# Pablete1234/parquet-floor

Measured on AMD Instinct MI355X. Metric: decoded GB/s + rows/s (node), lineitem-shape Snappy+dict, 1/2/4/8 GPUs, higher is better.
Workload: dtype u8; 1 GPU; lineitem SF1 x1 (6001215 rows x 1, 16 cols, 6 row groups of 1Mi rows), Snappy + dictionary, device-resident; row_groups_per_rank=6, compressed_page_bytes_rank0=217870360

## Files before the change

### parquet-floor_amd/csrc/pf_internal.h

```cpp
#pragma once
#include <stdint.h>

#include "pf_page_tables.h"

namespace pf {

struct Int2 {
    int x, y;
};

struct PfOpts {
    int exec = 5;
    bool ba_fused = true;
    bool page_null = false;
    int null_stagger = 0;
    bool nest_timeout = false;
    uint32_t null_dcap = 0;
    unsigned debug_skip = 0;
    int force_serial = 0;
    int force_redo = 0;
    bool zc = true;
    bool dl_kernel = true;
    bool h2d_kernel = false;
    int h2d_grid = 256;
    bool dl_stream = true;
    bool dl_prio = false;
    bool debug_plan = false;
    int64_t nest_seg = 0;
    bool nest_seg_set = false;
    bool dbp_par = true;
    bool bloom_first = true;
    bool flat_dstr = true;
    int fix_shift = 1;
};

constexpr uint32_t BA_TILE = 8192;
constexpr uint64_t BA_SHORT = 48;
constexpr uint32_t STICKY_DICT = 64u << 10;
constexpr uint32_t SNAP_RB = 128;
constexpr uint32_t SNAP_WIN = 64 * SNAP_RB;
constexpr uint32_t SNAP_WWORDS = SNAP_WIN / 32;
constexpr uint32_t SNAP_BLOCK = 65536;

struct SnapWin {
    uint32_t entry;
    uint32_t exit;
    uint32_t out;
    uint32_t flags;
};

struct SnapEnt {
    uint32_t pos;
    uint32_t out;
};

enum : int32_t {
    PG_V2 = 1,
    PG_COMPRESSED = 2,
    PG_DICT = 4,
};

struct SnappyJob {
    const uint8_t* src;
    uint8_t* dst;
    uint32_t src_len;
// ... 257 lines not shown
```

### parquet-floor_amd/csrc/pf_launch.h

```cpp
#pragma once
#include <hip/hip_runtime.h>

#include "pf_internal.h"
#include "pfloor.h"

namespace pf {

void launch_snappy_serial(const SnappyJob* d_jobs, int n_jobs, const int* d_fallback, DevChunkResult* d_res, hipStream_t s);
void launch_snappy_parse(const SnappyJob* d_jobs, int n_jobs, const int2* d_wins, int n_wins, SnapWin* d_win, SnapEnt* d_ent,
                         uint32_t* d_lane_out, uint32_t* d_splits, int* d_fb, int max_nwin, hipStream_t s);
void launch_snappy_exec(const SnappyJob* d_jobs, int n_jobs, const int2* d_pieces, int n_pieces, uint32_t* d_splits, int* d_fb,
                        DevChunkResult* d_res, int exec, hipStream_t s);
void launch_snappy(const SnappyJob* d_jobs, int n_jobs, const int2* d_wins, int n_wins, SnapWin* d_win, SnapEnt* d_ent,
                   uint32_t* d_lane_out, const int2* d_pieces, int n_pieces, uint32_t* d_splits, int* d_fb,
                   DevChunkResult* d_res, int max_nwin, int exec, hipStream_t s);
#ifdef PF_DIAG
void launch_snappy_exec2(const SnappyJob* d_jobs, int n_jobs, const int2* d_pieces, int n_pieces, const uint32_t* d_splits,
                         int* d_fb, hipStream_t s);
#endif

void launch_zstd(ZstdJob* d_jobs, const int* d_order, int n_jobs, uint8_t* d_lit, uint32_t lit_stride, DevChunkResult* d_res,
                 hipStream_t s);

void launch_lz4(Lz4Job* d_jobs, const int* d_order, int n_jobs, DevChunkResult* d_res, hipStream_t s);

void launch_snappy_head(SnappyJob* d_jobs, int n_jobs, DevPage* d_pages, const DevChunk* d_chunks, int* d_fb,
                        const DevChunkResult* d_res, hipStream_t st);
void launch_snappy_litcopy(const SnappyJob* d_jobs, const int* d_list, int n, const int* d_fb, hipStream_t st);

void launch_ba(BaJob* d_jobs, int n_jobs, const int2* d_tiles, int n_tiles, DevChunkResult* d_res, hipStream_t st,
               bool short_values);

void launch_runs(const DevChunk* d_chunks, DevPage* d_pages, const int* d_list, int n, DevChunkResult* d_res, hipStream_t st);
void launch_lvl(const DevChunk* d_chunks, DevPage* d_pages, const int* d_list, int n, DevChunkResult* d_res, hipStream_t st,
                bool page_null, NullCaps nc);
void launch_count_flat(const DevChunk* d_chunks, DevPage* d_pages, const int* d_list, int n, int n_flat, const int2* d_dblk,
                       int n_dblk, DevChunkResult* d_res, BaJob* d_bajobs, hipStream_t st);
void launch_flat(const DevChunk* d_chunks, DevPage* d_pages, const int* d_list, int nfix, int n, int n4, int n8, int* d_fbq,
                 const int2* d_dblk, int n_dblk, DevChunkResult* d_res, hipStream_t st, NullCaps nc, int stagger);

void launch_nest_lvl(const DevChunk* d_chunks, DevPage* d_pages, const int* d_list, int n, int max_nwin, DevChunkResult* d_res,
                     hipStream_t st, bool force_timeout);
void launch_count(const DevChunk* d_chunks, DevPage* d_pages, const int* d_list, int n, DevChunkResult* d_res, BaJob* d_bajobs,
                  hipStream_t st, int idle_grid);
void launch_nest_count(const DevChunk* d_chunks, DevPage* d_pages, const int* d_list, int n, const int2* d_segs, int n_segs,
                       DevChunkResult* d_res, hipStream_t st);
void launch_scan(DevChunk* d_chunks, DevPage* d_pages, const int* d_list, int n, DevChunkResult* d_res, uint8_t* arena,
                 uint64_t cap, unsigned long long* used, hipStream_t st);
// ... 24 lines not shown
```

### parquet-floor_amd/csrc/pf_runtime.hip

```cpp
#include <hip/hip_runtime.h>

#include <algorithm>
#include <chrono>
#include <cstdio>
#include <cstdlib>
#include <cstring>
#include <memory>
#include <mutex>
#include <string>
#include <vector>

#include "pf_ctx.h"
#include "pf_host.h"
#include "pf_launch.h"
#include "pf_plan.h"
#include "pf_snappy_par.h"
#include "pfloor.h"

using namespace pf;

static_assert(sizeof(Int2) == sizeof(int2) && alignof(Int2) <= alignof(int2), "the planner's pairs are the kernels' int2");

namespace {

// ... 68 lines not shown
    hipStream_t st = ctx->stream;
    const BatchPlan& p = ctx->plan;
    uint8_t* meta = static_cast<uint8_t*>(ctx->d_meta.p);
    DevChunk* d_chunks = reinterpret_cast<DevChunk*>(meta + p.off_chunks);
    DevPage* d_pages = reinterpret_cast<DevPage*>(meta + p.off_pages);
    SnappyJob* d_jobs = reinterpret_cast<SnappyJob*>(meta + p.off_jobs);
    DevChunkResult* d_res = reinterpret_cast<DevChunkResult*>(meta + p.off_res);
    auto list = [&](ListId l) { return reinterpret_cast<int*>(meta + p.off_lists) + p.list_base[l]; };
    auto pairs = [&](ListId l) { return reinterpret_cast<const int2*>(list(l)); };
    auto len = [&](ListId l) { return int(p.lists[l].size()); };
    const int n_jobs = int(p.jobs.size()), n_nest = len(L_NEST), n_nseg = len(L_NSEG) / 2;
    unsigned long long* used = reinterpret_cast<unsigned long long*>(meta + p.meta_bytes - 256);
    const int2* d_pieces = reinterpret_cast<const int2*>(meta + p.off_pieces);
    uint32_t* d_splits = reinterpret_cast<uint32_t*>(meta + p.off_splits);
    int* d_fallback = reinterpret_cast<int*>(meta + p.off_fallback);
    const int2* d_wins = reinterpret_cast<const int2*>(meta + p.off_wins);

#ifdef PF_DIAG
    const unsigned skip = ctx->opts.debug_skip;
#else
    constexpr unsigned skip = 0;
#endif
    if (!ctx->meta_by_kernel) {
        if (p.bits_bytes) HIPCHK(ctx, hipMemsetAsync(ctx->d_bits.p, 0, p.bits_bytes, st));
        if (p.npub_bytes) HIPCHK(ctx, hipMemsetAsync(static_cast<uint8_t*>(ctx->d_scratch.p) + p.off_npub, 0, p.npub_bytes, st));
    }
    EVREC(ctx, ctx->ev[1], st);
    if (!(skip & 1u)) launch_snappy_head(d_jobs, n_jobs, d_pages, d_chunks, d_fallback, d_res, st);
    if (!(skip & 1u)) launch_snappy_litcopy(d_jobs, list(L_DJOBS), len(L_DJOBS), d_fallback, st);
    if (!(skip & 1u)) launch_snappy_parse(d_jobs, n_jobs, d_wins, int(p.snap.wins.size()), p.snap.d_win, p.snap.d_ent,
                        p.snap.d_lane_out, d_splits, d_fallback, p.snap.max_snap_win, st);
    EVREC(ctx, ctx->ev[2], st);
    if (!(skip & 2u))
        launch_snappy_exec(d_jobs, n_jobs, d_pieces, int(p.snap.pieces.size()), d_splits, d_fallback, d_res, ctx->opts.exec, st);
    launch_zstd(reinterpret_cast<ZstdJob*>(meta + p.off_zjobs), list(L_ZSTD), int(p.zjobs.size()),
                static_cast<uint8_t*>(ctx->d_scratch.p) + p.off_zlit, p.zlit_stride, d_res, st);
    launch_lz4(reinterpret_cast<Lz4Job*>(meta + p.off_ljobs), list(L_LZ4), int(p.ljobs.size()), d_res, st);
    EVREC(ctx, ctx->ev[3], st);
    BaJob* d_bajobs = reinterpret_cast<BaJob*>(meta + p.off_bajobs);
    const int2* d_batiles = reinterpret_cast<const int2*>(meta + p.off_batiles);
    const int n_ba = int(p.bajobs.size()), n_bt = int(p.ba_tiles.size());
    if (!(skip & 4u)) launch_ba(d_bajobs, p.n_ba_dict, d_batiles, p.n_ba_dict_tiles, d_res, st, p.ba_short_dict && ctx->opts.ba_fused);
    EVREC(ctx, ctx->ev[4], st);
    launch_delta(d_chunks, d_pages, list(L_DELTA), len(L_DELTA), p.max_dbp_nwin, d_res, st);
    EVREC(ctx, ctx->ev[5], st);
    if (!(skip & 8u)) launch_runs(d_chunks, d_pages, list(L_RUNS), len(L_RUNS), d_res, st);
    NullCaps ncaps = p.null_caps;
    if (ctx->opts.null_dcap) ncaps.dcap = ctx->opts.null_dcap;
    if (!(skip & 8u)) launch_lvl(d_chunks, d_pages, list(L_LVL), len(L_LVL), d_res, st, ctx->opts.page_null, ncaps);
    launch_dlen(d_chunks, d_pages, list(L_DLEN), len(L_DLEN), d_res, st);
    EVREC(ctx, ctx->ev[6], st);
    launch_nest_lvl(d_chunks, d_pages, list(L_NEST), n_nest, p.max_nwin, d_res, st, ctx->opts.nest_timeout);
    if (!(skip & 16u)) {
        launch_count_flat(d_chunks, d_pages, list(L_COUNT), len(L_COUNT), p.n_count_flat, pairs(L_CDICT), len(L_CDICT) / 2,
                          d_res, d_bajobs, st);
        launch_count(d_chunks, d_pages, list(L_COUNT), len(L_COUNT), d_res, d_bajobs, st, COUNT_IDLE_GRID);
    }
    launch_nest_count(d_chunks, d_pages, list(L_NEST), n_nest, pairs(L_NSEG), n_nseg, d_res, st);
    if (!(skip & 4u))
        launch_ba(d_bajobs + p.n_ba_dict, n_ba - p.n_ba_dict, d_batiles + p.n_ba_dict_tiles, n_bt - p.n_ba_dict_tiles,
                  d_res, st, p.ba_short_data && ctx->opts.ba_fused);
    EVREC(ctx, ctx->ev[7], st);
    launch_scan(d_chunks, d_pages, list(L_SCAN), len(L_SCAN), d_res, static_cast<uint8_t*>(ctx->d_chars.p),
                ctx->d_chars.cap, used, st);
    EVREC(ctx, ctx->ev[8], st);
    if (!(skip & 32u))
        launch_flat(d_chunks, d_pages, list(L_FLAT), p.n_flat_fixed, p.n_flat_all, p.n_null4, p.n_null8,
// ... 126 lines not shown

namespace {
#ifdef PF_DIAG
void opts_from_env(pf::PfOpts& o) {
    auto on = [](const char* name, bool dflt) { const char* e = std::getenv(name); return e ? e[0] == '1' : dflt; };
    auto num = [](const char* name, int dflt) { const char* e = std::getenv(name); return e ? std::atoi(e) : dflt; };
    o.exec = num("PF_EXEC", o.exec);
    o.ba_fused = on("PF_BA_FUSED", o.ba_fused);
    o.page_null = on("PF_PAGE_NULL", o.page_null);
    o.nest_timeout = on("PF_DEBUG_NEST_TIMEOUT", o.nest_timeout);
    o.null_dcap = uint32_t(std::max(0, num("PF_NULL_DCAP", 0))) & ~15u;
    o.null_stagger = num("PF_DEBUG_NULL_STAGGER", o.null_stagger);
    if (const char* e = std::getenv("PF_DEBUG_SKIP")) {
        const char* names[] = {"parse", "exec", "ba", "levels", "count", "flat", "decode"};
        for (int i = 0; i < 7; i++)
            if (std::strstr(e, names[i])) o.debug_skip |= 1u << i;
    }
    o.force_serial = num("PF_DEBUG_FORCE_SERIAL", o.force_serial);
    o.force_redo = num("PF_DEBUG_FORCE_REDO", o.force_redo);
    o.zc = on("PF_ZC", o.zc);
    o.dl_kernel = on("PF_DL_KERNEL", o.dl_kernel);
    o.dl_stream = on("PF_DL_STREAM", o.dl_stream);
    o.h2d_kernel = on("PF_H2D_KERNEL", o.h2d_kernel);
    o.h2d_grid = std::max(1, num("PF_H2D_GRID", o.h2d_grid));
    o.dl_prio = on("PF_DL_PRIO", o.dl_prio);
    o.debug_plan = on("PF_DEBUG_PLAN", o.debug_plan);
    if (const char* e = std::getenv("PF_NEST_SEG")) {
        o.nest_seg = std::atoll(e);
        o.nest_seg_set = true;
    }
    o.dbp_par = on("PF_DBP_PAR", o.dbp_par);
    o.bloom_first = on("PF_BLOOM_FIRST", o.bloom_first);
    o.flat_dstr = on("PF_FLAT_DSTR", o.flat_dstr);
    const int fb = num("PF_FIX_BLK", 8192);
    o.fix_shift = fb >= 16384 ? 2 : (fb >= 8192 ? 1 : 0);
}
#endif

int ctx_init(pf_ctx* ctx, pf_ctx* peer) {
#ifdef PF_DIAG
    opts_from_env(ctx->opts);
#endif
    HIPCHK(nullptr, hipSetDevice(ctx->device));
    if (peer) {
        ctx->streams = peer->streams;
    } else {
        ctx->streams = std::make_shared<Streams>();
        ctx->streams->device = ctx->device;
        HIPCHK(nullptr, hipStreamCreateWithFlags(&ctx->streams->stream, hipStreamNonBlocking));
    }
    ctx->stream = ctx->streams->stream;
    ctx->zc = ctx->opts.zc;
    HIPCHK(nullptr, hipEventCreateWithFlags(&ctx->ev_done, hipEventDisableTiming));
    HIPCHK(nullptr, hipEventCreateWithFlags(&ctx->ev_copy, hipEventDisableTiming));
    HIPCHK(nullptr, hipEventCreateWithFlags(&ctx->ev_dl, hipEventDisableTiming));
    for (auto& e : ctx->ev) HIPCHK(nullptr, hipEventCreate(&e));
    for (auto& e : ctx->ev_bloom) HIPCHK(nullptr, hipEventCreate(&e));
    for (auto& e : ctx->ev_win) HIPCHK(nullptr, hipEventCreate(&e));
    for (auto& e : ctx->ev_sel) HIPCHK(nullptr, hipEventCreate(&e));
    return PF_OK;
}

int ctx_create(int device, pf_ctx* peer, pf_ctx** out) {
    pf_ctx* ctx = new pf_ctx();
    ctx->device = device;
    const int rc = ctx_init(ctx, peer);
// ... 495 lines not shown
    SnappyJob job{};
    job.src = static_cast<const uint8_t*>(ctx->d_in.p);
    job.dst = static_cast<uint8_t*>(ctx->d_scratch.p);
    job.src_len = uint32_t(n);
    job.dst_len = uint32_t(ulen);
    std::vector<SnappyJob> jobs(1, job);
    SnappyPlan sp;
    plan_snappy(jobs, sp);
    HIPCHK(ctx, ctx->d_tokmap.ensure(sp.tokmap_bytes));
    bind_snappy(jobs, sp, reinterpret_cast<uintptr_t>(ctx->d_tokmap.p));
    ctx->d_last_win = sp.d_win;
    ctx->d_last_lane_out = sp.d_lane_out;
    size_t m = 0;
    auto take = [](size_t& cursor, size_t sz) { size_t o = align_up(cursor, 256); cursor = o + sz; return o; };
    size_t o_job = take(m, sizeof(SnappyJob)), o_pc = take(m, sizeof(int2) * sp.pieces.size());
    size_t o_sp = take(m, 4 * sp.pieces.size()), o_fb = take(m, 4), o_wn = take(m, sizeof(int2) * sp.wins.size());
    size_t o_res = take(m, sizeof(DevChunkResult));
    m = align_up(m, 256);
    HIPCHK(ctx, ctx->d_meta.ensure(m));
    HIPCHK(ctx, ctx->h_meta.ensure(m));
    uint8_t* h = static_cast<uint8_t*>(ctx->h_meta.p);
    std::memset(h, 0, m);
    std::memcpy(h + o_job, jobs.data(), sizeof(SnappyJob));
    std::memcpy(h + o_pc, sp.pieces.data(), sizeof(int2) * sp.pieces.size());
    std::memset(h + o_sp, 0xff, 4 * sp.pieces.size());
    std::memcpy(h + o_wn, sp.wins.data(), sizeof(int2) * sp.wins.size());
    uint8_t* d = static_cast<uint8_t*>(ctx->d_meta.p);
    HIPCHK(ctx, hipMemcpyAsync(d, h, m, hipMemcpyHostToDevice, st));
    ctx->d_last_splits = reinterpret_cast<const uint32_t*>(d + o_sp);
    launch_snappy(reinterpret_cast<const SnappyJob*>(d + o_job), 1, reinterpret_cast<const int2*>(d + o_wn),
                  int(sp.wins.size()), sp.d_win, sp.d_ent, sp.d_lane_out, reinterpret_cast<const int2*>(d + o_pc),
                  int(sp.pieces.size()), reinterpret_cast<uint32_t*>(d + o_sp), reinterpret_cast<int*>(d + o_fb),
                  reinterpret_cast<DevChunkResult*>(d + o_res), int(jobs[0].n_win),
                  ctx->opts.exec, st);
    HIPCHK(ctx, hipGetLastError());
    HIPCHK(ctx, ctx->h_res.ensure(512));
    HIPCHK(ctx, hipMemcpyAsync(ctx->h_res.p, d + o_res, sizeof(DevChunkResult), hipMemcpyDeviceToHost, st));
    HIPCHK(ctx, hipMemcpyAsync(static_cast<uint8_t*>(ctx->h_res.p) + 256, d + o_fb, 4, hipMemcpyDeviceToHost, st));
    if (ulen) HIPCHK(ctx, hipMemcpyAsync(dst, ctx->d_scratch.p, ulen, hipMemcpyDeviceToHost, st));
    HIPCHK(ctx, hipStreamSynchronize(st));
    const DevChunkResult* r = static_cast<const DevChunkResult*>(ctx->h_res.p);
    if (r->status != 0) return fail(ctx, r->status, "snappy: corrupt input");
    return PF_OK;
}

int pf_zstd_decompress(pf_ctx* ctx, const uint8_t* src, size_t n, uint8_t* dst, size_t cap, size_t* out_len) {
    if (!ctx || (!src && n) || (!dst && cap) || !out_len) return fail(ctx, PF_ERR_INVALID_ARG, "null arg");
    if (ctx->pending) return fail(ctx, PF_ERR_STATE, "previous decode not waited for");
    if (n > (1ull << 30) || cap > (1ull << 30)) return fail(ctx, PF_ERR_INVALID_ARG, "zstd: buffer too large");
    *out_len = 0;
    if (const int rc = begin_oneshot(ctx, true)) return rc;
    hipStream_t st = ctx->stream;
    const uint32_t stride = zstd_lit_stride(uint32_t(cap));
    const size_t o_lit = align_up(cap + 16, 256);
    HIPCHK(ctx, ctx->d_in.ensure(std::max<size_t>(n, 1)));
    HIPCHK(ctx, ctx->d_scratch.ensure(o_lit + stride));
    if (n) HIPCHK(ctx, hipMemcpyAsync(ctx->d_in.p, src, n, hipMemcpyHostToDevice, st));
    ZstdJob job{};
    job.src = static_cast<const uint8_t*>(ctx->d_in.p);
    job.dst = static_cast<uint8_t*>(ctx->d_scratch.p);
    job.src_len = uint32_t(n);
    job.dst_len = uint32_t(cap);
    const size_t o_res = 256, m = 512;
    HIPCHK(ctx, ctx->d_meta.ensure(m));
    HIPCHK(ctx, ctx->h_meta.ensure(m));
    HIPCHK(ctx, ctx->h_res.ensure(512));
    uint8_t* h = static_cast<uint8_t*>(ctx->h_meta.p);
// ... 243 lines not shown
```

### parquet-floor_amd/csrc/pf_snappy_exec.hip

```cpp
#include <hip/hip_runtime.h>

#include "pf_launch.h"
#include "pf_snappy_exec.h"
#include "pf_stamps.h"

namespace pf {

#ifdef PF_STAMPS
PF_STAMP_TABLE(pf_stamps, 16, pf_debug_stamps)
#define STAMP_ADD(i, v) atomicAdd(&pf_stamps[i], (unsigned long long)(v))
#else
#define STAMP_ADD(i, v) ((void)0)
#endif

#ifndef PF_X5_BATCH
#define PF_X5_BATCH 764
#endif
constexpr uint32_t X5_BATCH = PF_X5_BATCH;
constexpr uint32_t X5_STG = (XSTAGE + 15u) & ~15u;
#ifndef PF_X5_FCH
#define PF_X5_FCH 64
#endif
constexpr uint32_t X5_FCH = PF_X5_FCH;
constexpr uint32_t X5_FSL = X5_FCH * 16u;
constexpr uint32_t X5_STAGE0 = XRING;
constexpr uint32_t X5_LDS = XRING + 2u * X5_STG;
constexpr uint32_t X5_W = 768u / 32u;
constexpr uint32_t X5_LINE = 128u;
#ifndef PF_X5_TPL
#define PF_X5_TPL 2
#endif
constexpr int X5_TPL = PF_X5_TPL;
constexpr uint32_t X5_DS = 64u * X5_TPL + 1u;
static_assert(X5_BATCH + 3u <= 768u, "a batch and its alignment bytes are at most three 256-byte windows");
static_assert(X5_FCH <= 128u, "a batch's far-copy chunks are loaded by at most two LDS-DMA wave instructions");
static_assert(X5_FCH >= 32u && (X5_FCH > 64u ? 128u : 64u) * 8u <= X5_FSL && (X5_FCH + 4u) * 8u <= X5_FSL,
              "the chunk address table (an entry per loading lane, and four past the last chunk) lies inside one batch's chunk bytes");
enum : uint32_t { R5_NORMAL = 0, R5_LONG = 1, R5_NOP = 2, R5_END = 3, R5_BAD = 4 };
constexpr uint32_t X5_CP = 0x80000000u;
static_assert(XRING <= 4096u, "ring-copy offsets must stay below 4096: tests/test_exec_arith.py checks (j * m) >> 16 up to there");

__device__ __forceinline__ void x5_barrier() { asm volatile("s_waitcnt lgkmcnt(0)\n\ts_barrier" ::: "memory"); }
__device__ __forceinline__ void x5_order() { asm volatile("" ::: "memory"); }

__device__ __forceinline__ uint32_t x5_pick(uint32_t w, uint32_t g) {
    uint32_t m, r;
    asm("v_pk_ashrrev_i16 %0, 15, %1 op_sel_hi:[0,1]" : "=v"(m) : "v"(w));
    asm("v_bfi_b32 %0, %1, %2, %3" : "=v"(r) : "v"(m), "v"(g), "v"(w));
    return r;
}

struct X5Lds {
    __attribute__((aligned(16))) uint8_t L[X5_LDS];
    uint16_t tokpos[XCHUNK / 2];
    uint32_t D[2][2 * X5_DS];
    uint32_t SB[2][X5_W], WP[2][X5_W];
    uint32_t REC[2][4];
    __attribute__((aligned(8))) uint16_t jv[256];
#if defined(PF_X5_PAD) && PF_X5_PAD > 0
    uint8_t pad[PF_X5_PAD];
#endif
};

__device__ __forceinline__ u32x4 x5_load16(const PF_GLOBAL uint8_t* gin, uint32_t src) {
    const uintptr_t a = reinterpret_cast<uintptr_t>(gin) + src;
    const PF_GLOBAL u32x4* p = (const PF_GLOBAL u32x4*)(a & ~uintptr_t(15));
    const uint32_t sh = uint32_t(a & 15u);
    const u32x4 A = p[0];
    u32x4 B = A;
    if (sh) B = p[1];
    const uint32_t w[8] = {A.x, A.y, A.z, A.w, B.x, B.y, B.z, B.w};
    const uint32_t k = sh >> 2, s = sh & 3u;
    u32x4 r;
    #pragma unroll
    for (int i = 0; i < 4; i++) {
        const uint32_t lo = k == 0 ? w[i] : (k == 1 ? w[i + 1] : (k == 2 ? w[i + 2] : w[i + 3]));
        const uint32_t hi = k == 0 ? w[i + 1] : (k == 1 ? w[i + 2] : (k == 2 ? w[i + 3] : w[i + 4]));
        r[i] = __builtin_amdgcn_alignbyte(hi, lo, s);
    }
    return r;
}

__device__ __forceinline__ void x5_dma16(uint64_t g, uint32_t lds) {
    asm volatile("s_mov_b32 m0, %1\n\ts_nop 0\n\tglobal_load_lds_dwordx4 %0, off" : : "v"(g), "s"(lds) : "memory");
}

static_assert(XSTAGE == 64u * 16u + 5u * 16u, "a staged chunk is 64 + 5 lane loads");
__device__ __forceinline__ void x5_chunk_load(const PF_GLOBAL uint8_t* gin, const PF_GLOBAL uint16_t* tm16, uint64_t n, uint32_t I,
                                              int lane, u32x4& va, u32x4& vb, uint32_t& bits) {
    const uintptr_t a = reinterpret_cast<uintptr_t>(gin + I);
    const uint32_t woff = uint32_t(a & 15u);
    const PF_GLOBAL u32x4* src = (const PF_GLOBAL u32x4*)(a - woff);
    const int64_t first = int64_t(I) - int64_t(woff);
    va = u32x4{0u, 0u, 0u, 0u};
    vb = u32x4{0u, 0u, 0u, 0u};
    bits = 0u;
    if (first + 16 * int64_t(lane) < int64_t(n)) va = src[lane];
    if (lane < 5 && first + 16 * int64_t(64 + lane) < int64_t(n)) vb = src[64 + lane];
    const uint32_t p16 = I + 16u * uint32_t(lane);
    if (uint64_t(p16) < n) bits = uint32_t(tm16[p16 >> 4]);
}

__device__ __forceinline__ void exec5_piece(X5Lds& S, uint8_t* FS, const SnappyJob* __restrict__ jobs, const int2* __restrict__ pieces,
                                            const uint32_t* __restrict__ splits, int* __restrict__ fb, int mode, int item) {
    uint8_t* const L = S.L;
    uint16_t* const tokpos = S.tokpos;
    auto& D = S.D;
    auto& SB = S.SB;
    auto& WP = S.WP;
    auto& REC = S.REC;
    uint8_t* const jvb = reinterpret_cast<uint8_t*>(S.jv);
    uint8_t* const ring = L;
    const uint32_t Lb = uint32_t(reinterpret_cast<uintptr_t>(L));
    const uint32_t FSB = uint32_t(reinterpret_cast<uintptr_t>(FS)) - Lb;
    const int wv = __builtin_amdgcn_readfirstlane(int(threadIdx.x) >> 6);
    const int lane = int(threadIdx.x) & 63;
    int j, k;
    if (mode == 0) {
        const int2 pc = pieces[item];
        j = pc.x;
        k = pc.y;
    } else {
        j = item;
        k = 0;
    }
    const int f = fb[j];
    bool whole;
    if (mode == 0) {
        if (f >= FB_REDO || (f == FB_WHOLE && k > 0)) return;
        whole = f == FB_WHOLE;
    } else {
        if (f != FB_REDO) return;
        whole = true;
    }
    const SnappyJob job = jobs[j];
    const uint8_t* in = job.src;
    const uint64_t n = job.src_len;
    const uint32_t* sp = splits + job.split_base;
    uint64_t pos0 = 0, ulen = 0;
    if (!uvarint(in, n, pos0, ulen) || ulen != job.dst_len) {
        if (threadIdx.x == 0) atomicMax(&fb[j], FB_SERIAL);
        return;
    }
    if (mode == 0 && (job.dflags & 1u)) {
        if (threadIdx.x == 0) atomicMax(&fb[j], FB_REDO);
        return;
    }
    uint32_t ip, out_start, out_end = job.dst_len;
    if (whole) {
        ip = uint32_t(pos0);
        out_start = 0;
    } else {
        if (k > 0 && sp[k] == SNAP_INVALID) return;
        ip = k == 0 ? uint32_t(pos0) : sp[k];
        out_start = uint32_t(k) * SNAP_BLOCK;
        for (uint32_t k2 = k + 1; k2 < job.n_pieces; k2++)
            if (sp[k2] != SNAP_INVALID) { out_end = k2 * SNAP_BLOCK; break; }
    }
    const PF_GLOBAL uint16_t* tm16 = (const PF_GLOBAL uint16_t*)(job.tokmap);
    const PF_GLOBAL uint8_t* gin = gptr(in);
    PF_GLOBAL uint8_t* gdst = gptr(job.dst);
    const OutDst od{gdst, mode == 0 ? gptr(job.ddst) : nullptr, job.dlo, job.dgran};
    if (threadIdx.x < 2) {
        D[threadIdx.x][0] = 0u;
        D[threadIdx.x][X5_DS] = 0u;
    }
    uint32_t op = out_start, sb = 0, T = 0, I = 0, woff = 0, cb = 1;
    uint32_t ops_m1 = out_start, k_m1 = R5_NOP, k_m2 = R5_NOP, nops = 0;
    uint32_t pfI = ~0u, pfbits = 0;
    u32x4 pfa = {0u, 0u, 0u, 0u}, pfb = {0u, 0u, 0u, 0u};
    uint32_t F = out_start, cop = out_start;
    uint32_t last = R5_END;
#ifdef PF_STAMPS
    unsigned long long x5t = __builtin_amdgcn_s_memtime();
#define X5T(i) do { const unsigned long long t_ = __builtin_amdgcn_s_memtime(); if (lane == 0) STAMP_ADD(i, t_ - x5t); x5t = t_; } while (0)
    if (threadIdx.x == 0) STAMP_ADD(13, 1);
#else
#define X5T(i) ((void)0)
#endif
    for (uint32_t it = 0;; it++) {
        const uint32_t b = it & 1u;
        if (wv == 0) {
            if (lane == 0) STAMP_ADD(12, 1);
            uint32_t kind = R5_BAD, b_op = op, b_tot = 0, b_s0 = 0;
            const uint32_t sf = out_start + ((ops_m1 - out_start) & ~(XSLOT - 1u));
            const uint32_t LF = k_m2 == R5_NORMAL ? (sf >= out_start + XSLOT ? sf - XSLOT : out_start) : sf;
            bool ok = true;
            if (op >= out_end) {
                kind = R5_END;
                ok = false;
            } else if (sb >= T) {
                if (ip >= n) {
                    ok = false;
                } else {
                    I = ip & ~15u;
                    cb ^= 1u;
                    u32x4 va, vb;
                    uint32_t bits;
                    if (I == pfI) {
                        va = pfa;
                        vb = pfb;
                        bits = pfbits;
                    } else {
                        x5_chunk_load(gin, tm16, n, I, lane, va, vb, bits);
                    }
                    u32x4* stq = reinterpret_cast<u32x4*>(L + X5_STAGE0 + cb * X5_STG);
                    stq[lane] = va;
                    if (lane < 5) stq[64 + lane] = vb;
                    woff = uint32_t(reinterpret_cast<uintptr_t>(gin + I) & 15u);
                    pfI = I + XCHUNK;
                    if (uint64_t(pfI) < n) x5_chunk_load(gin, tm16, n, pfI, lane, pfa, pfb, pfbits);
                    else pfI = ~0u;
                    const uint32_t p16 = I + 16u * uint32_t(lane);
                    if (p16 + 16u <= ip) bits = 0;
                    else if (p16 < ip) bits &= ~((1u << (ip - p16)) - 1u);
                    const uint32_t cnt = __popc(bits);
                    const uint32_t ex = dpp_incl_scan(cnt);
                    T = __builtin_amdgcn_readlane(ex, 63);
                    uint32_t q = ex - cnt;
                    while (bits) {
                        const uint32_t bb = uint32_t(__ffs(bits) - 1);
                        bits &= bits - 1;
                        tokpos[q++] = uint16_t(16u * uint32_t(lane) + bb);
                    }
                    sb = 0;
                    x5_order();
                    if (T == 0) ok = false;
                }
            }
            X5T(0);
            if (ok) {
                const uint32_t stg_off = __builtin_amdgcn_readfirstlane(cb) ? X5_STAGE0 + X5_STG : X5_STAGE0;
                const uint8_t* stg = L + stg_off;
                uint32_t pos[X5_TPL], ol[X5_TPL], start[X5_TPL], endp[X5_TPL], inc[X5_TPL], otok[X5_TPL];
                bool v[X5_TPL], take[X5_TPL];
                SnapTok32 tk[X5_TPL];
                #pragma unroll
                for (int h = 0; h < X5_TPL; h++) {
                    const uint32_t t = sb + 64u * uint32_t(h) + uint32_t(lane);
                    v[h] = t < T;
                    pos[h] = uint32_t(tokpos[min(t, XCHUNK / 2u - 1u)]);
                    if (!v[h]) pos[h] = 0u;
                }
                uint32_t tlo[X5_TPL], thi[X5_TPL];
                #pragma unroll
                for (int h = 0; h < X5_TPL; h++) lds_read8_2(stg, woff + pos[h], tlo[h], thi[h]);
                #pragma unroll
                for (int h = 0; h < X5_TPL; h++) tk[h] = snap_tok32(tlo[h], thi[h]);
                int nt = 0;
                bool wrong = false;
                uint32_t prevlast = ip, incbase = 0;
                #pragma unroll
                for (int h = 0; h < X5_TPL; h++) {
                    ol[h] = v[h] ? tk[h].ol : 0u;
                    start[h] = I + pos[h];
                    endp[h] = __builtin_elementwise_add_sat(start[h], tk[h].tl);
                    const uint32_t pdpp = dpp_prev(endp[h]);
                    const uint32_t prev = lane == 0 ? prevlast : pdpp;
                    inc[h] = incbase + dpp_incl_scan(ol[h]);
                    otok[h] = op + inc[h] - ol[h];
                    take[h] = v[h] && otok[h] < out_end;
                    nt += __popcll(__ballot(take[h]));
                    wrong = wrong || (take[h] && (start[h] != prev || endp[h] > n || op + inc[h] > out_end || inc[h] < ol[h] ||
                                                  inc[h] < incbase));
                    prevlast = __builtin_amdgcn_readlane(endp[h], 63);
                    incbase = __builtin_amdgcn_readlane(inc[h], 63);
                }
                if (__any(wrong) || nt == 0) {
                    ok = false;
                } else {
                    uint32_t kd[X5_TPL], off[X5_TPL], srcv[X5_TPL], a[X5_TPL], fsh[X5_TPL], nch[X5_TPL], fce[X5_TPL];
                    bool farc[X5_TPL], fnr[X5_TPL], lstaged[X5_TPL], fdd[X5_TPL];
                    unsigned long long cutm[X5_TPL], farm = 0;
                    unsigned long long wide2 = 0, wide4 = 0;
                    #pragma unroll
                    for (int h = 0; h < X5_TPL; h++) {
                        kd[h] = tk[h].kind;
                        off[h] = tk[h].arg;
                        srcv[h] = start[h] + tk[h].arg;
                        lstaged[h] = srcv[h] + ol[h] <= I + XCHUNK + 64;
                        a[h] = otok[h] - off[h];
                        farc[h] = take[h] && kd[h] != 0 && a[h] + min(ol[h], off[h]) <= op &&
                                  int32_t(a[h] - (op + X5_BATCH - XRING)) < 0;
                        fnr[h] = farc[h] && a[h] + ol[h] + (X5_LINE - 1u) > LF;
                        farm |= __ballot(farc[h]);
                        fsh[h] = 0u;
                        nch[h] = 0u;
                        fce[h] = 0u;
                        fdd[h] = false;
                    }
                    if (farm) {
                        const uint32_t dst_lo = uint32_t(reinterpret_cast<uintptr_t>(gdst)) & 15u;
                        const uint32_t dd_lo = uint32_t(reinterpret_cast<uintptr_t>(od.dd)) & 15u;
                        uint32_t anyn = 0;
                        #pragma unroll
                        for (int h = 0; h < X5_TPL; h++) {
                            fdd[h] = od.dd != nullptr && a[h] >= od.dlo;
                            fsh[h] = ((fdd[h] ? dd_lo : dst_lo) + a[h]) & 15u;
                            nch[h] = farc[h] ? (fsh[h] + ol[h] + 15u) >> 4 : 0u;
                            anyn |= nch[h];
                        }
                        wide2 = __ballot(anyn > 1u);
                        wide4 = __ballot(anyn > 3u);
                        uint32_t cbase = 0;
                        #pragma unroll
                        for (int h = 0; h < X5_TPL; h += 2) {
                            const int h1 = h + 1 < X5_TPL ? h + 1 : h;
                            const uint32_t sc = dpp_incl_scan(nch[h] | (h1 != h ? nch[h1] << 16 : 0u));
                            const uint32_t tot = __builtin_amdgcn_readlane(sc, 63);
                            fce[h] = cbase + (sc & 0xffffu);
                            cbase += tot & 0xffffu;
                            if (h1 != h) {
                                fce[h1] = cbase + (sc >> 16);
// ... 55 lines not shown
                                    const uint64_t fb0 = reinterpret_cast<uintptr_t>((fdd[h] ? od.dd : gdst) + a[h]) & ~uintptr_t(15);
                                    fb0v[h] = fb0;
                                }
                                #pragma unroll
                                for (int i = 4; i >= 0; i--) {
                                    if ((i >= 3 && !wide4) || (i >= 1 && !wide2)) continue;
                                    #pragma unroll
                                    for (int h = 0; h < X5_TPL; h++)
                                        if (far[h]) ca[fce[h] - nch[h] + uint32_t(i)] = fb0v[h] + 16u * uint32_t(i);
                                }
                                x5_order();
                                const uint32_t l0 = uint32_t(lane);
                                uint64_t s0a = ca[l0];
                                uint64_t s1a = 0;
                                if constexpr (X5_FCH > 64u)
                                    if (ntot > 64u) s1a = ca[64u + l0];
                                asm volatile("" : "+v"(s0a), "+v"(s1a) :: "memory");
                                uint8_t* chunks = FS + b * X5_FSL;
                                const uint32_t sl0 = __builtin_amdgcn_readfirstlane(uint32_t(reinterpret_cast<uintptr_t>(chunks)));
                                if (l0 < ntot) x5_dma16(s0a, sl0);
                                if constexpr (X5_FCH > 64u)
                                    if (ntot > 64u && l0 + 64u < ntot) x5_dma16(s1a, sl0 + 1024u);
                            }
                            X5T(2);
                            if (lane < int(X5_W)) SB[b][lane] = 0;
                            #pragma unroll
                            for (int h = 0; h < X5_TPL; h++) {
                                const uint32_t relS = otok[h] - (op & ~3u);
                                uint32_t d0 = 0, d1 = 0;
                                if (inb[h]) {
                                    const bool near = cp[h] && !far[h];
                                    d0 = relS | (near ? (X5_CP | (off[h] << 16)) : 0u);
                                    d1 = near ? uint32_t(65536.0f * __builtin_amdgcn_rcpf(float(off[h]))) + 1u
                                              : (lit[h] ? stg_off + woff + (srcv[h] - I) - relS
                                                        : FSB + b * X5_FSL + 16u * (fce[h] - nch[h]) + fsh[h] - relS);
                                }
                                D[b][1 + 64 * h + lane] = d0;
                                D[b][1 + X5_DS + 64 * h + lane] = d1;
                                x5_order();
                                if (inb[h]) atomicOr(&SB[b][relS >> 5], 1u << (relS & 31u));
                            }
                            x5_order();
                            const uint32_t c = lane < int(X5_W) ? __popc(SB[b][lane]) : 0u;
                            const uint32_t e2 = dpp_incl_scan(c) - c;
                            if (lane < int(X5_W)) WP[b][lane] = e2;
                            kind = R5_NORMAL;
                            b_tot = btot;
                            nops = 0;
                        }
                    }
                    if (ok && used) {
                        op += b_tot;
                        const uint32_t uh = (used - 1u) >> 6;
                        #pragma unroll
                        for (int h = 0; h < X5_TPL; h++)
                            if (uh == uint32_t(h)) ip = __builtin_amdgcn_readlane(endp[h], (used - 1u) & 63u);
                        sb += used;
                    }
                }
            }
            if (!ok && kind != R5_END) kind = R5_BAD;
            if (lane == 0) {
                REC[b][0] = kind;
                REC[b][1] = b_op;
                REC[b][2] = b_tot;
                REC[b][3] = b_s0;
            }
            asm volatile("s_waitcnt vmcnt(0)" ::: "memory");
            X5T(3);
            k_m2 = k_m1;
            k_m1 = kind;
            ops_m1 = b_op;
        } else if (it > 0) {
            const uint32_t pb = b ^ 1u;
            const uint32_t kind = __builtin_amdgcn_readfirstlane(REC[pb][0]);
            const uint32_t s0 = __builtin_amdgcn_readfirstlane(REC[pb][1]);
            const uint32_t btot = __builtin_amdgcn_readfirstlane(REC[pb][2]);
            if (kind == R5_NORMAL) {
                const uint32_t al = s0 & 3u;
                const uint32_t Sb = s0 - al;
                const uint32_t btS = btot + al;
                const uint32_t* sbw = SB[pb];
                const uint32_t* wpw = WP[pb];
                const uint32_t* Dp = D[pb];
                for (uint32_t w0 = 0; w0 < btS; w0 += 256) {
                    const uint32_t x0 = w0 + 4u * uint32_t(lane);
                    const uint32_t ws = w0 == 0 ? al : w0;
                    const uint32_t wd = x0 >> 5, sh = x0 & 31u;
                    const uint32_t sbv = sbw[wd];
                    const uint32_t t0 = wpw[wd] + __popc(sbv & ((2u << sh) - 1u));
                    const uint32_t nb = sbv >> sh;
                    uint32_t tk[4];
                    tk[0] = t0;
                    tk[1] = t0 + ((nb >> 1) & 1u);
// ... 67 lines not shown
                            for (uint32_t q = max(p, s0); q < min(p + 16u, e); q++) ring[q & XRMASK] = gin[sl + (q - s0)];
                        }
                    }
                    flush_slots(ring, od, F, min(base + XLIT, e), lane);
                }
                cop = e;
                wait_vmem();
            } else {
                wait_vmem();
            }
        }
        X5T(9);
        x5_barrier();
        if (wv == 0) X5T(4); else X5T(10);
        last = __builtin_amdgcn_readfirstlane(REC[b][0]);
        if (last >= R5_END) break;
    }
    if (last == R5_BAD) {
        if (threadIdx.x == 0) atomicMax(&fb[j], whole ? FB_SERIAL : FB_REDO);
        return;
    }
    if (wv == 1) {
        for (uint32_t a = F + uint32_t(lane) * 16u; a + 16u <= cop; a += 1024u)
            put16(od, a, *reinterpret_cast<const u32x4*>(ring + (a & XRMASK)));
        for (uint32_t a = F + ((cop - F) & ~15u) + uint32_t(lane); a < cop; a += 64) put1(od, a, ring[a & XRMASK]);
    }
#undef X5T
}

__global__ __launch_bounds__(128) void k_snappy_exec5(const SnappyJob* __restrict__ jobs, const int2* __restrict__ pieces,
                                                      const uint32_t* __restrict__ splits, int* __restrict__ fb, int mode) {
    __shared__ X5Lds S;
    __shared__ __attribute__((aligned(16))) uint8_t FS[2 * X5_FSL];
    exec5_piece(S, FS, jobs, pieces, splits, fb, mode, int(blockIdx.x));
}

void launch_snappy_exec(const SnappyJob* d_jobs, int n_jobs, const int2* d_pieces, int n_pieces, uint32_t* d_splits,
                        int* d_fb, DevChunkResult* d_res, int exec, hipStream_t s) {
    if (n_jobs <= 0) return;
#ifdef PF_DIAG
    if (exec == 2) {
        launch_snappy_exec2(d_jobs, n_jobs, d_pieces, n_pieces, d_splits, d_fb, s);
    } else
#else
    (void)exec;
#endif
    {
        hipLaunchKernelGGL(k_snappy_exec5, dim3(n_pieces), dim3(128), 0, s, d_jobs, d_pieces, (const uint32_t*)d_splits, d_fb, 0);
        hipLaunchKernelGGL(k_snappy_exec5, dim3(n_jobs), dim3(128), 0, s, d_jobs, d_pieces, (const uint32_t*)d_splits, d_fb, 1);
    }
    launch_snappy_serial(d_jobs, n_jobs, d_fb, d_res, s);
}

void launch_snappy(const SnappyJob* d_jobs, int n_jobs, const int2* d_wins, int n_wins, SnapWin* d_win,
                   SnapEnt* d_ent, uint32_t* d_lane_out, const int2* d_pieces, int n_pieces, uint32_t* d_splits,
                   int* d_fb, DevChunkResult* d_res, int max_nwin, int exec, hipStream_t s) {
    launch_snappy_parse(d_jobs, n_jobs, d_wins, n_wins, d_win, d_ent, d_lane_out, d_splits, d_fb, max_nwin, s);
    launch_snappy_exec(d_jobs, n_jobs, d_pieces, n_pieces, d_splits, d_fb, d_res, exec, s);
}

}
```

Before: 416.9 decoded GB/s.

## Let Snappy exec5 batches span two staged input chunks

When fewer than a full batch of tokens remain in the current staged chunk, the exec5 decoder now stages the next chunk into the other buffer. It carries the leftover token positions over and enumerates the next chunk's tokens into an extended tokpos array. Batches can then straddle the chunk boundary instead of issuing a short, underfilled batch. The aim is fewer underutilized wave batches and fewer chunk-reload stalls. In exchange it adds more LDS for tokpos, more control logic, and hazard tracking that holds a batch when a buffer is still in use.

Result: no change. 419.2 decoded GB/s, median of 6 (+0.6%).

```diff
diff --git a/parquet-floor_amd/csrc/pf_internal.h b/parquet-floor_amd/csrc/pf_internal.h
--- a/parquet-floor_amd/csrc/pf_internal.h
+++ b/parquet-floor_amd/csrc/pf_internal.h
@@ -31,6 +31,7 @@
     bool dbp_par = true;
     bool bloom_first = true;
     bool flat_dstr = true;
+    bool x5_span = true;
     int fix_shift = 1;
 };
 
diff --git a/parquet-floor_amd/csrc/pf_launch.h b/parquet-floor_amd/csrc/pf_launch.h
--- a/parquet-floor_amd/csrc/pf_launch.h
+++ b/parquet-floor_amd/csrc/pf_launch.h
@@ -10,10 +10,10 @@
 void launch_snappy_parse(const SnappyJob* d_jobs, int n_jobs, const int2* d_wins, int n_wins, SnapWin* d_win, SnapEnt* d_ent,
                          uint32_t* d_lane_out, uint32_t* d_splits, int* d_fb, int max_nwin, hipStream_t s);
 void launch_snappy_exec(const SnappyJob* d_jobs, int n_jobs, const int2* d_pieces, int n_pieces, uint32_t* d_splits, int* d_fb,
-                        DevChunkResult* d_res, int exec, hipStream_t s);
+                        DevChunkResult* d_res, int exec, bool span, hipStream_t s);
 void launch_snappy(const SnappyJob* d_jobs, int n_jobs, const int2* d_wins, int n_wins, SnapWin* d_win, SnapEnt* d_ent,
                    uint32_t* d_lane_out, const int2* d_pieces, int n_pieces, uint32_t* d_splits, int* d_fb,
-                   DevChunkResult* d_res, int max_nwin, int exec, hipStream_t s);
+                   DevChunkResult* d_res, int max_nwin, int exec, bool span, hipStream_t s);
 #ifdef PF_DIAG
 void launch_snappy_exec2(const SnappyJob* d_jobs, int n_jobs, const int2* d_pieces, int n_pieces, const uint32_t* d_splits,
                          int* d_fb, hipStream_t s);
diff --git a/parquet-floor_amd/csrc/pf_runtime.hip b/parquet-floor_amd/csrc/pf_runtime.hip
--- a/parquet-floor_amd/csrc/pf_runtime.hip
+++ b/parquet-floor_amd/csrc/pf_runtime.hip
@@ -124,7 +124,7 @@
                         p.snap.d_lane_out, d_splits, d_fallback, p.snap.max_snap_win, st);
     EVREC(ctx, ctx->ev[2], st);
     if (!(skip & 2u))
-        launch_snappy_exec(d_jobs, n_jobs, d_pieces, int(p.snap.pieces.size()), d_splits, d_fallback, d_res, ctx->opts.exec, st);
+        launch_snappy_exec(d_jobs, n_jobs, d_pieces, int(p.snap.pieces.size()), d_splits, d_fallback, d_res, ctx->opts.exec, ctx->opts.x5_span, st);
     launch_zstd(reinterpret_cast<ZstdJob*>(meta + p.off_zjobs), list(L_ZSTD), int(p.zjobs.size()),
                 static_cast<uint8_t*>(ctx->d_scratch.p) + p.off_zlit, p.zlit_stride, d_res, st);
     launch_lz4(reinterpret_cast<Lz4Job*>(meta + p.off_ljobs), list(L_LZ4), int(p.ljobs.size()), d_res, st);
@@ -317,6 +317,7 @@
     o.dbp_par = on("PF_DBP_PAR", o.dbp_par);
     o.bloom_first = on("PF_BLOOM_FIRST", o.bloom_first);
     o.flat_dstr = on("PF_FLAT_DSTR", o.flat_dstr);
+    o.x5_span = on("PF_X5_SPAN", o.x5_span);
     const int fb = num("PF_FIX_BLK", 8192);
     o.fix_shift = fb >= 16384 ? 2 : (fb >= 8192 ? 1 : 0);
 }
@@ -878,7 +879,7 @@
                   int(sp.wins.size()), sp.d_win, sp.d_ent, sp.d_lane_out, reinterpret_cast<const int2*>(d + o_pc),
                   int(sp.pieces.size()), reinterpret_cast<uint32_t*>(d + o_sp), reinterpret_cast<int*>(d + o_fb),
                   reinterpret_cast<DevChunkResult*>(d + o_res), int(jobs[0].n_win),
-                  ctx->opts.exec, st);
+                  ctx->opts.exec, ctx->opts.x5_span, st);
     HIPCHK(ctx, hipGetLastError());
     HIPCHK(ctx, ctx->h_res.ensure(512));
     HIPCHK(ctx, hipMemcpyAsync(ctx->h_res.p, d + o_res, sizeof(DevChunkResult), hipMemcpyDeviceToHost, st));
diff --git a/parquet-floor_amd/csrc/pf_snappy_exec.hip b/parquet-floor_amd/csrc/pf_snappy_exec.hip
--- a/parquet-floor_amd/csrc/pf_snappy_exec.hip
+++ b/parquet-floor_amd/csrc/pf_snappy_exec.hip
@@ -32,6 +32,12 @@
 #endif
 constexpr int X5_TPL = PF_X5_TPL;
 constexpr uint32_t X5_DS = 64u * X5_TPL + 1u;
+constexpr uint32_t X5_TOK = XCHUNK / 2u + 64u * X5_TPL;
+constexpr uint32_t X5_SPMIN = 16u;
+constexpr uint32_t X5_LSKIP = 5u + 64u - 1u;
+static_assert(64u * X5_TPL - 1u + XCHUNK / 2u <= X5_TOK, "a leftover below one batch's tokens and a whole chunk's tokens fit");
+static_assert((XCHUNK & (XCHUNK - 1u)) == 0u && 2u * XCHUNK <= 65536u, "bit XCHUNK of a 16-bit position tells the chunk");
+static_assert(X5_STG % 16u == 0u && X5_STG >= XCHUNK + 64u + 16u, "a stage buffer holds a chunk, a 64-byte literal past it and the alignment");
 static_assert(X5_BATCH + 3u <= 768u, "a batch and its alignment bytes are at most three 256-byte windows");
 static_assert(X5_FCH <= 128u, "a batch's far-copy chunks are loaded by at most two LDS-DMA wave instructions");
 static_assert(X5_FCH >= 32u && (X5_FCH > 64u ? 128u : 64u) * 8u <= X5_FSL && (X5_FCH + 4u) * 8u <= X5_FSL,
@@ -52,7 +58,7 @@
 
 struct X5Lds {
     __attribute__((aligned(16))) uint8_t L[X5_LDS];
-    uint16_t tokpos[XCHUNK / 2];
+    uint16_t tokpos[X5_TOK];
     uint32_t D[2][2 * X5_DS];
     uint32_t SB[2][X5_W], WP[2][X5_W];
     uint32_t REC[2][4];
@@ -101,8 +107,35 @@
     if (uint64_t(p16) < n) bits = uint32_t(tm16[p16 >> 4]);
 }
 
+__device__ __forceinline__ uint32_t x5_enum(uint16_t* tokpos, uint32_t bits, int lane, uint32_t q0, uint32_t pbase) {
+    const uint32_t cnt = __popc(bits);
+    const uint32_t ex = dpp_incl_scan(cnt);
+    uint32_t q = q0 + ex - cnt;
+    while (bits) {
+        const uint32_t bb = uint32_t(__ffs(bits) - 1);
+        bits &= bits - 1;
+        tokpos[q++] = uint16_t(pbase + 16u * uint32_t(lane) + bb);
+    }
+    return __builtin_amdgcn_readlane(ex, 63);
+}
+
+#if defined(PF_DIAG) && !defined(PF_STAMPS)
+__device__ unsigned long long pf_x5_counts[3];
+extern "C" int pf_debug_x5_counts(unsigned long long* out, int reset) {
+    if (hipMemcpyFromSymbol(out, HIP_SYMBOL(pf_x5_counts), sizeof(unsigned long long) * 3) != hipSuccess) return -1;
+    if (reset) {
+        const unsigned long long z[3] = {0, 0, 0};
+        if (hipMemcpyToSymbol(HIP_SYMBOL(pf_x5_counts), z, sizeof z) != hipSuccess) return -1;
+    }
+    return 0;
+}
+#define X5_COUNT(i) (lane == 0 ? (void)atomicAdd(&pf_x5_counts[i], 1ull) : (void)0)
+#else
+#define X5_COUNT(i) ((void)0)
+#endif
+
 __device__ __forceinline__ void exec5_piece(X5Lds& S, uint8_t* FS, const SnappyJob* __restrict__ jobs, const int2* __restrict__ pieces,
-                                            const uint32_t* __restrict__ splits, int* __restrict__ fb, int mode, int item) {
+                                            const uint32_t* __restrict__ splits, int* __restrict__ fb, int mode, int item, bool span) {
     uint8_t* const L = S.L;
     uint16_t* const tokpos = S.tokpos;
     auto& D = S.D;
@@ -167,6 +200,7 @@
     }
     uint32_t op = out_start, sb = 0, T = 0, I = 0, woff = 0, cb = 1;
     uint32_t ops_m1 = out_start, k_m1 = R5_NOP, k_m2 = R5_NOP, nops = 0;
+    uint32_t two = 0, Tn = 0, m1mask = 0;
     uint32_t pfI = ~0u, pfbits = 0;
     u32x4 pfa = {0u, 0u, 0u, 0u}, pfb = {0u, 0u, 0u, 0u};
     uint32_t F = out_start, cop = out_start;
@@ -185,13 +219,23 @@
             uint32_t kind = R5_BAD, b_op = op, b_tot = 0, b_s0 = 0;
             const uint32_t sf = out_start + ((ops_m1 - out_start) & ~(XSLOT - 1u));
             const uint32_t LF = k_m2 == R5_NORMAL ? (sf >= out_start + XSLOT ? sf - XSLOT : out_start) : sf;
-            bool ok = true;
+            uint32_t bmask = 0;
+            bool ok = true, hold = false;
             if (op >= out_end) {
                 kind = R5_END;
                 ok = false;
             } else if (sb >= T) {
+                if (two) {
+                    I += XCHUNK;
+                    cb ^= 1u;
+                    two = 0;
+                }
                 if (ip >= n) {
                     ok = false;
+                } else if ((m1mask >> (cb ^ 1u)) & 1u) {
+                    hold = true;
+                    kind = R5_NOP;
+                    X5_COUNT(2);
                 } else {
                     I = ip & ~15u;
                     cb ^= 1u;
@@ -214,37 +258,68 @@
                     const uint32_t p16 = I + 16u * uint32_t(lane);
                     if (p16 + 16u <= ip) bits = 0;
                     else if (p16 < ip) bits &= ~((1u << (ip - p16)) - 1u);
-                    const uint32_t cnt = __popc(bits);
-                    const uint32_t ex = dpp_incl_scan(cnt);
-                    T = __builtin_amdgcn_readlane(ex, 63);
-                    uint32_t q = ex - cnt;
-                    while (bits) {
-                        const uint32_t bb = uint32_t(__ffs(bits) - 1);
-                        bits &= bits - 1;
-                        tokpos[q++] = uint16_t(16u * uint32_t(lane) + bb);
-                    }
+                    T = x5_enum(tokpos, bits, lane, 0u, 0u);
                     sb = 0;
                     x5_order();
                     if (T == 0) ok = false;
                 }
+            } else if (span && T - sb < 64u * uint32_t(X5_TPL) && (!two || sb >= Tn) && pfI == I + (two ? 2u * XCHUNK : XCHUNK) &&
+                       T - (two ? Tn : 0u) >= X5_SPMIN) {
+                const unsigned long long bm = __ballot(pfbits != 0u);
+                bool lskip = true;
+                if (bm) {
+                    const uint32_t l0 = uint32_t(__ffsll(bm) - 1);
+                    const uint32_t b0 = __builtin_amdgcn_readlane(pfbits, l0);
+                    lskip = 16u * l0 + uint32_t(__ffs(b0) - 1) > X5_LSKIP;
+                }
+                if (lskip) {
+                } else if ((m1mask >> (two ? cb : cb ^ 1u)) & 1u) {
+                    X5_COUNT(2);
+                } else {
+                    const uint32_t left = T - sb, rebase = two ? XCHUNK : 0u;
+                    if (two) {
+                        I += XCHUNK;
+                        cb ^= 1u;
+                    }
+                    uint32_t lp[X5_TPL];
+                    #pragma unroll
+                    for (int h = 0; h < X5_TPL; h++) lp[h] = uint32_t(tokpos[min(sb + 64u * uint32_t(h) + uint32_t(lane), X5_TOK - 1u)]);
+                    x5_order();
+                    #pragma unroll
+                    for (int h = 0; h < X5_TPL; h++)
+                        if (64u * uint32_t(h) + uint32_t(lane) < left) tokpos[64 * h + lane] = uint16_t(lp[h] - rebase);
+                    u32x4* stq = reinterpret_cast<u32x4*>(L + X5_STAGE0 + (cb ^ 1u) * X5_STG);
+                    stq[lane] = pfa;
+                    if (lane < 5) stq[64 + lane] = pfb;
+                    const uint32_t bits = pfbits;
+                    pfI = I + 2u * XCHUNK;
+                    if (uint64_t(pfI) < n) x5_chunk_load(gin, tm16, n, pfI, lane, pfa, pfb, pfbits);
+                    else pfI = ~0u;
+                    T = left + x5_enum(tokpos, bits, lane, left, XCHUNK);
+                    Tn = left;
+                    two = 1;
+                    sb = 0;
+                    x5_order();
+                }
             }
             X5T(0);
-            if (ok) {
+            if (ok && !hold) {
                 const uint32_t stg_off = __builtin_amdgcn_readfirstlane(cb) ? X5_STAGE0 + X5_STG : X5_STAGE0;
-                const uint8_t* stg = L + stg_off;
-                uint32_t pos[X5_TPL], ol[X5_TPL], start[X5_TPL], endp[X5_TPL], inc[X5_TPL], otok[X5_TPL];
+                const uint32_t sdel = (__builtin_amdgcn_readfirstlane(cb) ? 0u - X5_STG : X5_STG) - XCHUNK;
+                uint32_t pos[X5_TPL], sadj[X5_TPL], ol[X5_TPL], start[X5_TPL], endp[X5_TPL], inc[X5_TPL], otok[X5_TPL];
                 bool v[X5_TPL], take[X5_TPL];
                 SnapTok32 tk[X5_TPL];
                 #pragma unroll
                 for (int h = 0; h < X5_TPL; h++) {
                     const uint32_t t = sb + 64u * uint32_t(h) + uint32_t(lane);
                     v[h] = t < T;
-                    pos[h] = uint32_t(tokpos[min(t, XCHUNK / 2u - 1u)]);
+                    pos[h] = uint32_t(tokpos[min(t, X5_TOK - 1u)]);
                     if (!v[h]) pos[h] = 0u;
+                    sadj[h] = pos[h] >= XCHUNK ? sdel : 0u;
                 }
                 uint32_t tlo[X5_TPL], thi[X5_TPL];
                 #pragma unroll
-                for (int h = 0; h < X5_TPL; h++) lds_read8_2(stg, woff + pos[h], tlo[h], thi[h]);
+                for (int h = 0; h < X5_TPL; h++) lds_read8_2(L, stg_off + woff + pos[h] + sadj[h], tlo[h], thi[h]);
                 #pragma unroll
                 for (int h = 0; h < X5_TPL; h++) tk[h] = snap_tok32(tlo[h], thi[h]);
                 int nt = 0;
@@ -278,7 +353,7 @@
                         kd[h] = tk[h].kind;
                         off[h] = tk[h].arg;
                         srcv[h] = start[h] + tk[h].arg;
-                        lstaged[h] = srcv[h] + ol[h] <= I + XCHUNK + 64;
+                        lstaged[h] = srcv[h] + ol[h] <= I + XCHUNK + 64 + (pos[h] & XCHUNK);
                         a[h] = otok[h] - off[h];
                         farc[h] = take[h] && kd[h] != 0 && a[h] + min(ol[h], off[h]) <= op &&
                                   int32_t(a[h] - (op + X5_BATCH - XRING)) < 0;
@@ -400,7 +475,7 @@
                                     const bool near = cp[h] && !far[h];
                                     d0 = relS | (near ? (X5_CP | (off[h] << 16)) : 0u);
                                     d1 = near ? uint32_t(65536.0f * __builtin_amdgcn_rcpf(float(off[h]))) + 1u
-                                              : (lit[h] ? stg_off + woff + (srcv[h] - I) - relS
+                                              : (lit[h] ? stg_off + woff + (srcv[h] - I) + sadj[h] - relS
                                                         : FSB + b * X5_FSL + 16u * (fce[h] - nch[h]) + fsh[h] - relS);
                                 }
                                 D[b][1 + 64 * h + lane] = d0;
@@ -418,6 +493,11 @@
                         }
                     }
                     if (ok && used) {
+                        if (kind == R5_NORMAL) {
+                            if (!two || sb < Tn) bmask |= 1u << cb;
+                            if (two && sb + used > Tn) bmask |= 2u >> cb;
+                            if (bmask == 3u) X5_COUNT(1);
+                        }
                         op += b_tot;
                         const uint32_t uh = (used - 1u) >> 6;
                         #pragma unroll
@@ -428,6 +508,8 @@
                 }
             }
             if (!ok && kind != R5_END) kind = R5_BAD;
+            if (kind != R5_END) X5_COUNT(0);
+            m1mask = bmask;
             if (lane == 0) {
                 REC[b][0] = kind;
                 REC[b][1] = b_op;
@@ -561,31 +643,38 @@
                                                       const uint32_t* __restrict__ splits, int* __restrict__ fb, int mode) {
     __shared__ X5Lds S;
     __shared__ __attribute__((aligned(16))) uint8_t FS[2 * X5_FSL];
-    exec5_piece(S, FS, jobs, pieces, splits, fb, mode, int(blockIdx.x));
+#ifdef PF_DIAG
+    exec5_piece(S, FS, jobs, pieces, splits, fb, mode & 1, int(blockIdx.x), !(mode & 2));
+#else
+    exec5_piece(S, FS, jobs, pieces, splits, fb, mode, int(blockIdx.x), true);
+#endif
 }
 
 void launch_snappy_exec(const SnappyJob* d_jobs, int n_jobs, const int2* d_pieces, int n_pieces, uint32_t* d_splits,
-                        int* d_fb, DevChunkResult* d_res, int exec, hipStream_t s) {
+                        int* d_fb, DevChunkResult* d_res, int exec, bool span, hipStream_t s) {
     if (n_jobs <= 0) return;
 #ifdef PF_DIAG
+    const int ns = span ? 0 : 2;
     if (exec == 2) {
         launch_snappy_exec2(d_jobs, n_jobs, d_pieces, n_pieces, d_splits, d_fb, s);
     } else
 #else
     (void)exec;
+    (void)span;
+    const int ns = 0;
 #endif
     {
-        hipLaunchKernelGGL(k_snappy_exec5, dim3(n_pieces), dim3(128), 0, s, d_jobs, d_pieces, (const uint32_t*)d_splits, d_fb, 0);
-        hipLaunchKernelGGL(k_snappy_exec5, dim3(n_jobs), dim3(128), 0, s, d_jobs, d_pieces, (const uint32_t*)d_splits, d_fb, 1);
+        hipLaunchKernelGGL(k_snappy_exec5, dim3(n_pieces), dim3(128), 0, s, d_jobs, d_pieces, (const uint32_t*)d_splits, d_fb, ns);
+        hipLaunchKernelGGL(k_snappy_exec5, dim3(n_jobs), dim3(128), 0, s, d_jobs, d_pieces, (const uint32_t*)d_splits, d_fb, ns | 1);
     }
     launch_snappy_serial(d_jobs, n_jobs, d_fb, d_res, s);
 }
 
 void launch_snappy(const SnappyJob* d_jobs, int n_jobs, const int2* d_wins, int n_wins, SnapWin* d_win,
                    SnapEnt* d_ent, uint32_t* d_lane_out, const int2* d_pieces, int n_pieces, uint32_t* d_splits,
-                   int* d_fb, DevChunkResult* d_res, int max_nwin, int exec, hipStream_t s) {
+                   int* d_fb, DevChunkResult* d_res, int max_nwin, int exec, bool span, hipStream_t s) {
     launch_snappy_parse(d_jobs, n_jobs, d_wins, n_wins, d_win, d_ent, d_lane_out, d_splits, d_fb, max_nwin, s);
-    launch_snappy_exec(d_jobs, n_jobs, d_pieces, n_pieces, d_splits, d_fb, d_res, exec, s);
-}
-
-}
+    launch_snappy_exec(d_jobs, n_jobs, d_pieces, n_pieces, d_splits, d_fb, d_res, exec, span, s);
+}
+
+}
```
